# catniplab/vjf

Hardware: AMD Instinct MI355X
Metric: trial-timesteps/sec (higher is better)
Workload: dtype f32

## Files before the change

vjf_amd/csrc/vjf_chol_kernel.h:

```cpp
#pragma once
#include <hip/hip_runtime.h>
#include "vjf_gram_kernel.h"
#include "vjf_plan.h"

#define VJF_CHOL_THREADS 512
#define VJF_CHOL_MAXBLK 7
#define VJF_PREP_ROWS 1

struct VjfPrepArgs {
    float* state;
    const float* red;
    float* gbuf;
    float* aux;
    float* loss4;
    int B_total;
    unsigned flags;
    int n_rowblk, n_sgdblk;
    const unsigned* wait_count;
    unsigned wait_target;
    int bid0;
    const unsigned* run_word; unsigned run_epoch;
    const unsigned* start_count; unsigned start_target;
    unsigned* done_count;
    unsigned* replay_mask; float* replay_rho; int replay_pass;
// ... 569 lines not shown
}

template <int DZP>
__device__ __forceinline__ void vjf_chol_body(const VjfPlan& P, const VjfCholArgs& A, float* lds, int* s_dead, const unsigned it_epoch,
                                              const float* it_red, const unsigned it_wait_target, const unsigned it_stat_target,
                                              const bool it_src_state) {
    int tid = threadIdx.x;
    asm volatile("" : "+v"(tid));
    const int lane = tid & 63, wave = tid >> 6;
    const int n = P.n, dz = P.dz;
    const int nbl = (n + 31) / 32, npad = nbl * 32, ntri = nbl * (nbl + 1) / 2;
    float* S = A.state;
    float* SC = S + P.off[VJF_SLOT_SCALARS];
    const bool do_upd = A.flags & VJF_FLAG_UPDATE, warm = A.flags & VJF_FLAG_WARM_UP;
    if (!do_upd) return;
    if (A.post && warm) return;
    if (A.post && !A.self_prep && tid == 0) __hip_atomic_store(A.flags_out + VJF_CHOL_MAXBLK + 2, it_epoch, __ATOMIC_RELAXED, __HIP_MEMORY_SCOPE_AGENT);
    float* s_blk = lds;
    float* s_aux = s_blk + (size_t)ntri * 1024;
    float* s_g = s_aux + (size_t)nbl * 1024;
    int* s_flag = (int*)(s_g + (size_t)npad * DZP * (DZP <= 16 ? 1 : 2));
    double* s_d = (double*)(s_flag + 8);
    int* s_bi = s_flag + 64;
    int* s_bj = s_bi + 32;

    float* Wm = S + P.off[VJF_SLOT_W_MEAN];
    float* Wc = S + P.off[VJF_SLOT_W_CHOL];
    float* Pm = S + P.off[VJF_SLOT_W_PREC];
    float* Lm = S + P.off[VJF_SLOT_W_PCHOL];
    const float* G = it_red + P.red_G;
    const float* FDX = it_red + P.red_FDX;
    float sig = S[P.off[VJF_SLOT_TR_LOGVAR]];
    const float Bf = (float)A.B_total;
    unsigned st = 0;
    const bool sp = A.post && A.self_prep;
    VJF_STAMP(0);
    if (tid < ntri) {
        int bi = 0;
        while ((bi + 1) * (bi + 2) / 2 <= tid) ++bi;
        s_bi[tid] = bi;
        s_bj[tid] = tid - bi * (bi + 1) / 2;
    }
    if (tid == 0) s_flag[0] = 1;
    if (tid < 16) s_flag[128 + tid] = 0;
    __syncthreads();
    auto stat_wait = [&]() {
        if (A.stat_count && (!vjf_wg_wait_sc1(A.stat_count, it_stat_target, tid, SC + VJF_SC_STATUS, (A.flags & VJF_FLAG_HANDOFF_ACQUIRE) != 0u) || (A.inject_epoch && tid == 0 && it_epoch == A.inject_epoch))) {
            vjf_status_or(SC + VJF_SC_STATUS, VJF_STATUS_RLS_FAILED | VJF_STATUS_WAIT_STATS);
            *s_dead = 1;
        }
    };
    if (warm) stat_wait();

    if (!warm) {
        auto diag_chain = [&](int k) {
            float* dk = s_blk + (size_t)vtri(k, k) * 1024;
            const bool good = potrf_inv_chain2(dk, s_aux + (size_t)k * 1024, lane, min(32, n - 32 * k));
            if (!good && lane == 0) s_flag[0] = 0;
            return good;
        };
        bool chain_good = true;
        auto pad4 = [](int gi, int gj) {
            return make_float4(gi == gj ? 1.f : 0.f, gi == gj + 1 ? 1.f : 0.f, gi == gj + 2 ? 1.f : 0.f, gi == gj + 3 ? 1.f : 0.f);
        };
        bool lscr_guard = false;
        auto sigma_wait = [&]() {
            asm volatile("s_waitcnt vmcnt(0)" ::: "memory");
            __syncthreads();
            if (tid == 0) __hip_atomic_store(A.flags_out + VJF_CHOL_MAXBLK + 2, it_epoch, __ATOMIC_RELAXED, __HIP_MEMORY_SCOPE_AGENT);
            vjf_chaos(tid, A.wait_count, 1);
            if (A.sig_word && it_wait_target != 0u) {
                if (tid == 0) {
                    bool there = false;
                    unsigned bits = 0u;
                    for (unsigned spins = 0; spins < VJF_WAIT_SPINS; ++spins) {
                        const unsigned long long v = __hip_atomic_load(A.sig_word, __ATOMIC_RELAXED, __HIP_MEMORY_SCOPE_AGENT);
                        if ((unsigned)(v >> 32) == it_epoch - 1u) { there = true; bits = (unsigned)v; break; }
                        if ((spins & 255u) == 255u && vjf_abort_seen(SC + VJF_SC_STATUS)) break;
                        __builtin_amdgcn_s_sleep(1);
                    }
                    s_flag[2] = (int)bits; s_flag[3] = there ? 1 : 0;
                }
                __syncthreads();
                sig = __uint_as_float((unsigned)s_flag[2]);
                if (!s_flag[3] && tid == 0) { vjf_status_or(SC + VJF_SC_STATUS, VJF_STATUS_RLS_FAILED | VJF_STATUS_WAIT_SIGMA); *s_dead = 1; }
                lscr_guard = true;
                return;
            }
            if (!vjf_wg_wait_sc1(A.wait_count, it_wait_target, tid, SC + VJF_SC_STATUS, (A.flags & VJF_FLAG_HANDOFF_ACQUIRE) != 0u)) { vjf_status_or(SC + VJF_SC_STATUS, VJF_STATUS_RLS_FAILED | VJF_STATUS_WAIT_SIGMA); *s_dead = 1; }
            sig = __hip_atomic_load(S + P.off[VJF_SLOT_TR_LOGVAR], __ATOMIC_RELAXED, __HIP_MEMORY_SCOPE_AGENT);
        };
        typedef unsigned chol_u4 __attribute__((ext_vector_type(4)));
        const __amdgpu_buffer_rsrc_t r_G = __builtin_amdgcn_make_buffer_rsrc(const_cast<float*>(G), 0, 0x7fffffff, 0x00020000);
        auto g4 = [&](int gi, int gj) {
            if (!(gi < n && gj < n)) return make_float4(0.f, 0.f, 0.f, 0.f);
            if (A.stat_count) {
                const chol_u4 v4 = __builtin_amdgcn_raw_buffer_load_b128(r_G, (gi * n + gj) * 4, 0, 16);
                return make_float4(__uint_as_float(v4[0]), __uint_as_float(v4[1]), __uint_as_float(v4[2]), __uint_as_float(v4[3]));
            }
            return *reinterpret_cast<const float4*>(G + (size_t)gi * n + gj);
        };
        constexpr int NT = VJF_CHOL_THREADS - 64, NQ = ((VJF_CHOL_MAXBLK * (VJF_CHOL_MAXBLK + 1) / 2 - 1) * 256 + NT - 1) / NT;
        const int t2 = tid - 64;
        float4 v[NQ], g[NQ];
        auto idx_of = [&](int q) { return wave == 0 ? (q < 4 ? lane + 64 * q : ntri * 256) : 256 + t2 + q * NT; };
#pragma unroll
        for (int q = 0; q < NQ; ++q) {
            const int idx = idx_of(q);
            v[q] = make_float4(0.f, 0.f, 0.f, 0.f); g[q] = v[q];
            if (idx < ntri * 256) {
                const int b = idx >> 8, r = (idx >> 3) & 31, c4 = (idx & 7) * 4;
                const int gi = s_bi[b] * 32 + r, gj = s_bj[b] * 32 + c4;
                if (sp && !it_src_state) v[q] = *reinterpret_cast<const float4*>(A.pscr + (size_t)idx * 4);
                else v[q] = (gi < n && gj < n) ? *reinterpret_cast<const float4*>(Pm + (size_t)gi * n + gj) : pad4(gi, gj);
            }
        }
        stat_wait();
        if (sp) {
#pragma unroll
            for (int q = 0; q < NQ; ++q) {
                const int idx = idx_of(q);
                if (idx < ntri * 256) {
                    const int b = idx >> 8, r = (idx >> 3) & 31, c4 = (idx & 7) * 4;
                    g[q] = g4(s_bi[b] * 32 + r, s_bj[b] * 32 + c4);
                }
            }
        }
        if (sp) {
            sigma_wait();
            const float inv_v = expf(-sig);
#pragma unroll
            for (int q = 0; q < NQ; ++q) {
                v[q].x = fmaf(g[q].x, inv_v, v[q].x); v[q].y = fmaf(g[q].y, inv_v, v[q].y);
                v[q].z = fmaf(g[q].z, inv_v, v[q].z); v[q].w = fmaf(g[q].w, inv_v, v[q].w);
            }
        }
#pragma unroll
        for (int q = 0; q < NQ; ++q) {
            const int idx = idx_of(q);
            if (idx < ntri * 256) {
                const int b = idx >> 8, r = (idx >> 3) & 31, c4 = (idx & 7) * 4;
                float* blk = s_blk + (size_t)b * 1024;
                blk[vsw(r, c4)] = v[q].x; blk[vsw(r, c4 + 1)] = v[q].y; blk[vsw(r, c4 + 2)] = v[q].z; blk[vsw(r, c4 + 3)] = v[q].w;
                if (A.post) *reinterpret_cast<float4*>(A.pscr + (size_t)idx * 4) = v[q];
            }
        }
        if (wave == 0) chain_good = diag_chain(0);
        else if (!A.post)
            for (int e = t2; e < npad * DZP; e += NT) {
                const int r = e / DZP, j = e - r * DZP;
                s_g[e] = (r < n && j < dz) ? A.gbuf[(size_t)r * dz + j] : 0.f;
            }
        __syncthreads();
        VJF_STAMP(1);

        auto trail = [&](int k, int t) {
            const int bi = k + 1 + s_bi[t], bj = k + 1 + s_bj[t];
            float* cb = s_blk + (size_t)vtri(bi, bj) * 1024;
            vjf_f32x16 acc;
            blk_load(acc, cb, lane);
            blk_mma<true>(acc, s_blk + (size_t)vtri(bi, k) * 1024, s_blk + (size_t)vtri(bj, k) * 1024, -1.f, lane);
            blk_store(acc, cb, lane);
        };
        auto put_block = [&](const float* blk, float* dst, int ld, int gi0, int gj0, bool lower_only) {
#pragma unroll
            for (int q = 0; q < 4; ++q) {
                const int idx = lane + 64 * q, r = idx >> 3, c4 = (idx & 7) * 4;
                vjf_f32x4 o;
                o[0] = (!lower_only || c4 <= r) ? blk[vsw(r, c4)] : 0.f;
                o[1] = (!lower_only || c4 + 1 <= r) ? blk[vsw(r, c4 + 1)] : 0.f;
                o[2] = (!lower_only || c4 + 2 <= r) ? blk[vsw(r, c4 + 2)] : 0.f;
                o[3] = (!lower_only || c4 + 3 <= r) ? blk[vsw(r, c4 + 3)] : 0.f;
                if (gi0 + r < ld && gj0 + c4 < ld) {
                    float* p = dst + (size_t)(gi0 + r) * ld + gj0 + c4;
                    asm volatile("global_store_dwordx4 %0, %1, off sc1\n\ts_nop 1" ::"v"(p), "v"(o) : "memory");
                }
            }
        };
        auto publish = [&](int k0, int k1, unsigned fail) {
            vjf_chaos(lane, A.flags_out + k0, 2);
            asm volatile("s_waitcnt vmcnt(0)" ::: "memory");
            if (lane >= k0 && lane < k1) __hip_atomic_store(A.flags_out + lane, (it_epoch << 1) | fail, __ATOMIC_RELAXED, __HIP_MEMORY_SCOPE_AGENT);
        };
        volatile int* s_ctl = s_flag + 128;
        enum { C_CHAIN = 0, C_P1 = 1, C_A = 2, C_B = 3, C_HB = 4 };
        volatile int* v_ok = s_flag;
        auto lds_wait = [&](int w, int target) {
            for (unsigned spins = 0; spins < (1u << 22); ++spins) {
                if (s_ctl[w] >= target || !v_ok[0]) break;
                __builtin_amdgcn_s_sleep(1);
            }
            if (s_ctl[w] < target && v_ok[0]) v_ok[0] = 0;
            __builtin_amdgcn_fence(__ATOMIC_ACQUIRE, "workgroup");
        };
        auto lds_post = [&](int w, int v) {
            __builtin_amdgcn_fence(__ATOMIC_RELEASE, "workgroup");
            if (lane == 0) s_ctl[w] = v;
        };
        auto hb_arrive = [&](int hw, int stages_done) {
            __builtin_amdgcn_fence(__ATOMIC_RELEASE, "workgroup");
            if (lane == 0) s_ctl[C_HB + hw] = stages_done;
        };
        auto hb_wait = [&](int stages_done) {
            for (unsigned spins = 0; spins < (1u << 22); ++spins) {
                int lo = s_ctl[C_HB];
#pragma unroll
                for (int h2 = 1; h2 < 6; ++h2) lo = min(lo, (int)s_ctl[C_HB + h2]);
                if (lo >= stages_done || !v_ok[0]) break;
                __builtin_amdgcn_s_sleep(1);
            }
            __builtin_amdgcn_fence(__ATOMIC_ACQUIRE, "workgroup");
        };
        auto panel_tile = [&](int bi, int k) {
            float* pb = s_blk + (size_t)vtri(bi, k) * 1024;
            vjf_f32x16 acc;
#pragma unroll
            for (int r = 0; r < 16; ++r) acc[r] = 0.f;
            blk_mma<true>(acc, pb, s_aux + (size_t)k * 1024, 1.f, lane);
            blk_store(acc, pb, lane);
        };
        auto trail_tile = [&](int bi, int bj, int k) {
            float* cb = s_blk + (size_t)vtri(bi, bj) * 1024;
            vjf_f32x16 acc;
            blk_load(acc, cb, lane);
            blk_mma<true>(acc, s_blk + (size_t)vtri(bi, k) * 1024, s_blk + (size_t)vtri(bj, k) * 1024, -1.f, lane);
            blk_store(acc, cb, lane);
        };
        int kdone = 0;
        if (wave == 0) {
            auto wait_ab = [&](int target) {
// ... 341 lines not shown
```

vjf_amd/csrc/vjf_mega_kernel.h:

```cpp
#pragma once
#include <hip/hip_runtime.h>
#include "vjf_chol_kernel.h"
#include "vjf_plan.h"
#include "vjf_post_kernel.h"
#include "vjf_trial_mfma_kernel.h"
#include "vjf_act.h"

#define VJF_MG_THREADS 512
#define VJF_MG_WAVES 8
#define VJF_MG_TR 32
#define VJF_MG_LD 33
#define VJF_MG_GROWS 96
#define VJF_MG_MAXQ 4
#define VJF_MG_RING 32
#define VJF_MG_TAG_TILES 512
#define RS_RESID 5

#ifndef MG_C_SPREAD
#define MG_C_SPREAD 1
#endif
enum {
    MG_C_FWD = 16 * MG_C_SPREAD,
    MG_C_K1 = 32 * MG_C_SPREAD,
    MG_C_BWD = 48 * MG_C_SPREAD,
// ... 759 lines not shown
                v2a += __shfl_xor(v2a, 16, 64); v2a += __shfl_xor(v2a, 32, 64);
                v2b += __shfl_xor(v2b, 16, 64); v2b += __shfl_xor(v2b, 32, 64);
                if (lane < 16) { s_red[wave * TR + lane] = v2a; s_red[wave * TR + 16 + lane] = v2b; }
                if (wave < nsl) {
                    const int sl = msl;
                    vjf_f32x4 acc0 = {0.f, 0.f, 0.f, 0.f}, acc1 = {0.f, 0.f, 0.f, 0.f};
                    if (mpre) { if (mke > mkb) mg_mma2_mm16(acc0, acc1, am, s_phi, dz, 0, mkb, mke, 0, lane); }
                    else mg_mma2(acc0, acc1, Wm, dz, dz, 0, s_phi, mkb, mke, lane);
                    float* pr = s_part + (size_t)(sl * 16 + 4 * (lane >> 4)) * LD + (lane & 15);
#pragma unroll
                    for (int r = 0; r < 4; ++r) { pr[r * LD] = acc0[r]; pr[r * LD + 16] = acc1[r]; }
                }
                mean_nsl = nsl;
            }
            __syncthreads(); MG_PHASE();
            };
            auto moments_b = [&]() {
            if (!replay) {
                if (tid < TR) {
                    float v = 0.f;
                    for (int w = 0; w < NW; ++w) v += s_red[w * TR + tid];
                    s_plv[tid] = logf(v);
                }
                for (int e = tid; e < TR * dz; e += NT) {
                    const int j = e >> 5, b = e & 31;
                    float v = 0.f;
                    for (int sl = 0; sl < mean_nsl; ++sl) v += s_part[(size_t)(sl * 16 + j) * LD + b];
                    s_pm[j * LD + b] = s_xu[j * LD + b] + v;
                    if (want_resid) s_dmu[j * LD + b] = v;
                }
            }
            __syncthreads(); MG_PHASE();
            };
            if (!RLS && !replay && first && !use_mom) { mg_warm(A.xt, P.n * P.n, wg, tid); mg_warm(S + P.off[VJF_SLOT_W_MEAN], (P.n * P.dz) & ~3, wg, tid); }
            if (!RLS && !replay && !use_mom) { moments_a(); moments_b(); }
            if (!RLS && !replay && first) VJF_MG_STAMPW(2);
            if (first && !replay) {
                if (gated) gate();
                if (gated && t > 0 && vjf_abort_wg()) return;
                if (want_replay) break;
                if (t > 0 && !tl) {
                    mg_warm(A.aux, P.aux_len, wg, tid);
                    mg_warm(S + P.train_off, P.train_len, wg, tid);
                }
            }
            float4 wv[2];
            const bool warm_now = first && !replay && rls_now && !rls_in;
            if (first && !replay) rho = mg_ld(S + P.off[VJF_SLOT_LIK_LOGVAR]);
            if (first && !replay && !mode_rls) sig = mg_ld(S + P.off[VJF_SLOT_TR_LOGVAR]);
            if (warm_now) {
                mg_warm_issue(A.xt, P.n * P.n, wg, tid, wv);
                sig = mg_ld(S + P.off[VJF_SLOT_TR_LOGVAR]);
                tri = mg_ld(SCW + VJF_SC_TRI_CLEAN) != 0.f;
                rls_in = true;
            }
            if (first && tl && !replay && t == 0) {
                if (!vjf_wg_wait_sc1<RLS ? VJF_POLL_SLEEP : VJF_POLL_SLEEP_LITE>(cnt + MG_C_IMG, (unsigned)A.n_sgd, tid, SCW + VJF_SC_STATUS, (A.flags & VJF_FLAG_HANDOFF_ACQUIRE) != 0u))
                    vjf_status_or(SCW + VJF_SC_STATUS, VJF_STATUS_RLS_FAILED | VJF_STATUS_WAIT_GATE);
                if (vjf_abort_wg()) return;
            }
            if (first && tl && !replay && (gated || t == 0)) {
                const __amdgpu_buffer_rsrc_t r_img = mg_rsrc(A.img);
                float4* dst = reinterpret_cast<float4*>(smem + Lo.th0);
                const int n4 = Lo.th_len >> 2;
                for (int q0 = tid; q0 < n4; q0 += 8 * NT) {
                    float4 v[8];
#pragma unroll
                    for (int q = 0; q < 8; ++q) if (q0 + q * NT < n4) v[q] = mg_ld4(r_img, (q0 + q * NT) * 4);
#pragma unroll
                    for (int q = 0; q < 8; ++q) if (q0 + q * NT < n4) dst[q0 + q * NT] = v[q];
                }
                __syncthreads(); MG_PHASE();
            }
            if (warm_now) mg_warm_retire(wv);
            if (first) { VJF_MG_STAMP(1); VJF_MG_STAMPX(27, -1); VJF_MG_STAMPW(0); }
            if (first && A.stamps && tid == 0 && t == A.T - 1 && !replay) {
                unsigned xcc;
                unsigned hwid;
                asm volatile("s_getreg_b32 %0, hwreg(HW_REG_XCC_ID)" : "=s"(xcc));
                asm volatile("s_getreg_b32 %0, hwreg(HW_REG_HW_ID)" : "=s"(hwid));
                A.stamps[1024 + (size_t)wg * 8 + 6] = (xcc & 15u) | ((unsigned long long)hwid << 8);
                A.stamps[1024 + (size_t)wg * 8 + 7] = rls_in ? 1u : 0u;
            }
            {
                const float* xin = s_in;
                int kin = din, aoff = 0;
                for (int l = 0; l < P.L; ++l) {
                    const float* WT = A.aux + P.aux_recT[l];
                    int th_w = 0, th_ldw = 0, th_b = 0;
                    if (tl) mg_theta_layer(P, Lo.th0, l, th_w, th_ldw, th_b);
                    const float* bias_l = smem + th_b; const float* bias_g = S + P.off[VJF_SLOT_REC_B0 + 2 * l];
                    float* out = s_act + aoff * LD;
                    const int hl = P.h[l], mt = (hl + 15) >> 4;
                    for (int tt = wave; tt < mt; tt += NW) {
                        vjf_f32x4 acc0 = {0.f, 0.f, 0.f, 0.f}, acc1 = {0.f, 0.f, 0.f, 0.f};
                        if (tl) mg_mma2_lds<false>(acc0, acc1, smem + th_w, th_ldw, hl, tt * 16, xin, 0, kin, lane);
                        else mg_mma2(acc0, acc1, WT, hl, hl, tt * 16, xin, 0, kin, lane);
#pragma unroll
                        for (int r = 0; r < 4; ++r) {
                            const int f = tt * 16 + 4 * (lane >> 4) + r;
                            if (f < hl) {
                                const float bf = tl ? ((mg_lds_cf*)bias_l)[f] : ((mg_glb_cf*)bias_g)[f];
                                if (ACT) {
                                    out[f * LD + (lane & 15)] = vjf_act_fwd(act, acc0[r] + bf);
                                    out[f * LD + 16 + (lane & 15)] = vjf_act_fwd(act, acc1[r] + bf);
                                } else {
                                    out[f * LD + (lane & 15)] = mg_tanh(acc0[r] + bf);
                                    out[f * LD + 16 + (lane & 15)] = mg_tanh(acc1[r] + bf);
                                }
                            }
                        }
                    }
                    __syncthreads(); MG_PHASE();
                    xin = out; kin = hl; aoff += hl;
                }
                if (first) VJF_MG_STAMP(23);
                const float* HT = A.aux + P.aux_headT;
                const int mt = (2 * dz + 15) >> 4;
                const int nsl = min(NW / mt, part_rows / (16 * mt));
                if (wave < mt * nsl) {
                    const int tt = wave / nsl, sl = wave - tt * nsl;
                    const int per = (((kin + 3) >> 2) + nsl - 1) / nsl * 4;
                    vjf_f32x4 acc0 = {0.f, 0.f, 0.f, 0.f}, acc1 = {0.f, 0.f, 0.f, 0.f};
                    if (tl) mg_mma2_lds<false>(acc0, acc1, smem + Lo.th_head, Lo.th_ldh, 2 * dz, tt * 16, xin, sl * per, min(kin, (sl + 1) * per), lane);
                    else mg_mma2(acc0, acc1, HT, 2 * dz, 2 * dz, tt * 16, xin, sl * per, min(kin, (sl + 1) * per), lane);
                    float* pr = s_part + (size_t)((sl * mt + tt) * 16 + 4 * (lane >> 4)) * LD + (lane & 15);
#pragma unroll
                    for (int r = 0; r < 4; ++r) { pr[r * LD] = acc0[r]; pr[r * LD + 16] = acc1[r]; }
                }
                __syncthreads(); MG_PHASE();
                if (first) VJF_MG_STAMP(24);
                const float* bl_l = smem + Lo.th_bl; const float* bl_g = S + P.off[VJF_SLOT_LV_B];
                for (int e = tid; e < TR * 2 * dz; e += NT) {
                    const int f = e >> 5, b = e & 31;
                    float v = 0.f;
                    for (int sl = 0; sl < nsl; ++sl) v += s_part[(size_t)((sl * mt + (f >> 4)) * 16 + (f & 15)) * LD + b];
                    if (f < dz) s_mu[f * LD + b] = v; else s_lv[(f - dz) * LD + b] = v + (tl ? ((mg_lds_cf*)bl_l)[f - dz] : ((mg_glb_cf*)bl_g)[f - dz]);
                }
            }
            __syncthreads(); MG_PHASE();
            if (first) VJF_MG_STAMP(3);
            for (int e = tid; e < TR * dz; e += NT) {
                const int j = e >> 5, b = e & 31;
                const float xt = fmaf(s_e2[j * LD + b], expf(0.5f * s_lv[j * LD + b]), s_mu[j * LD + b]);
                s_xt[j * LD + b] = xt;
                s_dx[j * LD + b] = b < nb ? xt - s_xu[j * LD + b] : 0.f;
            }
            if (!replay) {
                float* mrow = mu_t + (size_t)b0 * dz;
                float* lrow = lv_t + (size_t)b0 * dz;
                const int ne = nb * dz;
                const int n4 = ((((size_t)mrow | (size_t)lrow) & 15u) == 0) ? (ne >> 2) : 0;
                for (int e4 = tid; e4 < n4; e4 += NT) {
                    float vm[4], vl[4];
#pragma unroll
                    for (int c = 0; c < 4; ++c) {
                        const int e = 4 * e4 + c, b = mg_div(e, m_dz), j = e - b * dz;
                        vm[c] = s_mu[j * LD + b]; vl[c] = s_lv[j * LD + b];
                    }
                    mg_st4(mrow + 4 * e4, vm[0], vm[1], vm[2], vm[3]);
                    mg_st4(lrow + 4 * e4, vl[0], vl[1], vl[2], vl[3]);
                }
                for (int e = 4 * n4 + tid; e < ne; e += NT) {
                    const int b = mg_div(e, m_dz), j = e - b * dz;
                    mg_st(mrow + e, s_mu[j * LD + b]);
                    mg_st(lrow + e, s_lv[j * LD + b]);
                }
            }
            __syncthreads(); MG_PHASE();
            {
                constexpr int LPT = NT / TR;
                const int b = tid / LPT, sl = tid % LPT;
                float sdx2 = 0.f;
                for (int j = sl; j < dz; j += LPT) { const float dx = s_dx[j * LD + b]; sdx2 = fmaf(dx, dx, sdx2); }
                sdx2 = group_sum<LPT>(sdx2);
                if (sl == 0) s_sc[b * RS_N + RS_SDX2] = sdx2;
            }
            {
                const float* CT = A.aux + P.aux_decT;
                const float* d_l = smem + Lo.th_bd; const float* d_g = S + P.off[VJF_SLOT_DEC_B];
                const int mt = (dy + 15) >> 4;
                for (int tt = wave; tt < mt; tt += NW) {
                    vjf_f32x4 acc0 = {0.f, 0.f, 0.f, 0.f}, acc1 = {0.f, 0.f, 0.f, 0.f};
                    if (tl) mg_mma2_lds<false>(acc0, acc1, smem + Lo.th_dec, Lo.th_ldd, dy, tt * 16, s_xt, 0, dz, lane);
                    else mg_mma2(acc0, acc1, CT, dy, dy, tt * 16, s_xt, 0, dz, lane);
#pragma unroll
                    for (int r = 0; r < 4; ++r) {
                        const int f = tt * 16 + 4 * (lane >> 4) + r;
                        if (f < dy) { const float df = tl ? ((mg_lds_cf*)d_l)[f] : ((mg_glb_cf*)d_g)[f]; s_py[f * LD + (lane & 15)] = acc0[r] + df; s_py[f * LD + 16 + (lane & 15)] = acc1[r] + df; }
                    }
                }
            }
            if (first) VJF_MG_STAMP(25);
            if (!replay && mode_rls) {
                const int mt = (n + 15) >> 4;
                for (int tt = NW - 1 - wave; tt < mt; tt += NW) {
                    const int m0 = tt * 16, i = lane & 15, kk = lane >> 4;
                    const float* arow = ((m0 + i) < n ? s_phi + (size_t)(m0 + i) * LD : s_zero) + kk;
                    const float* brow = (i < dz ? s_dx + (size_t)i * LD : s_zero) + kk;
                    float a[8], b[8];
#pragma unroll
                    for (int s = 0; s < 8; ++s) { a[s] = arow[4 * s]; b[s] = brow[4 * s]; }
                    vjf_f32x4 acc = {0.f, 0.f, 0.f, 0.f}, acc1 = {0.f, 0.f, 0.f, 0.f};
#pragma unroll
                    for (int s = 0; s < 8; s += 2) {
                        acc = __builtin_amdgcn_mfma_f32_16x16x4f32(a[s], b[s], acc, 0, 0, 0);
                        acc1 = __builtin_amdgcn_mfma_f32_16x16x4f32(a[s + 1], b[s + 1], acc1, 0, 0, 0);
                    }
                    acc += acc1;
                    const int fq = m0 + 4 * (lane >> 4), col = lane & 15;
                    if (col < dz && fq < ldn) {
                        float* p = early + (size_t)col * ldn + fq;
                        if (!first) { acc[0] += mg_ld(p); acc[1] += mg_ld(p + 1); acc[2] += mg_ld(p + 2); acc[3] += mg_ld(p + 3); }
                        mg_st4(p, acc[0], acc[1], acc[2], acc[3]);
                    }
                }
            }
            if (tid == 0 && first && last && !replay && !rls_in)
                s_wg[15] = ((int)(__hip_atomic_load(cnt + MG_C_PDONE, __ATOMIC_RELAXED, __HIP_MEMORY_SCOPE_AGENT) - (unsigned)t * npost) >= 0) ? 1.f : 0.f;
            if (use_mom && !replay) asm volatile("s_waitcnt vmcnt(0)" ::: "memory");
            __syncthreads(); MG_PHASE();
            if (use_mom && !replay && tid == 0) __hip_atomic_store(cnt + MG_C_TAG_POST + tile, (unsigned)(tc + 1), __ATOMIC_RELAXED, __HIP_MEMORY_SCOPE_AGENT);
            float touch = 0.f;
            if (!gated && !replay && last && tc + 1 < A.T) {
                const int tn = wg;
                const int b0n = tn * TR, nbn = min(TR, A.B - b0n);
                const int ly = (nbn * dy + 31) / 32 + 1, le = (nbn * dz + 31) / 32 + 1;
                const float* yn = A.y + (size_t)(tc + 1) * sy + (size_t)b0n * dy;
                const float* en = A.eps + (size_t)(tc + 1) * 2 * sz + (size_t)b0n * dz;
                const float* tp = nullptr;
                if (tid < ly) tp = yn + min(tid * 32, nbn * dy - 1);
                else if (tid < ly + le) tp = en + min((tid - ly) * 32, nbn * dz - 1);
                else if (tid < ly + 2 * le) tp = en + sz + min((tid - ly - le) * 32, nbn * dz - 1);
                if (tp) touch = *tp;
            }
            if (tid == 0 && !replay && mode_rls) {
                float v = 0.f;
                for (int bb = 0; bb < TR; ++bb) v += s_sc[bb * RS_N + RS_SDX2];
                s_wg[RS_SDX2] += v;
                if (last) mg_st(early + (size_t)16 * ldn + RS_SDX2, s_wg[RS_SDX2]);
            }
            if (first) VJF_MG_STAMP(26);
            const bool fuse_fwd = first && last && !replay && !rls_in && s_wg[15] != 0.f;
            if (last && !replay && !fuse_fwd && mode_rls) vjf_wg_signal_wt(cnt + MG_C_FWD, tid);
            if (first) VJF_MG_STAMP(4);
            if (last) { VJF_MG_STAMPX(28, -1); VJF_MG_STAMPW(1); }
            float4 wv_late[2];
            bool warm_late = false;
            if (first && !rls_in) {
                if (!vjf_wg_wait_sc1<RLS ? VJF_POLL_SLEEP : VJF_POLL_SLEEP_LITE>(cnt + MG_C_PDONE, (unsigned)t * npost, tid, SCW + VJF_SC_STATUS, (A.flags & VJF_FLAG_HANDOFF_ACQUIRE) != 0u))
                    vjf_status_or(SCW + VJF_SC_STATUS, VJF_STATUS_RLS_FAILED | VJF_STATUS_WAIT_K1);
                if (vjf_abort_wg()) return;
                sig = mg_ld(S + P.off[VJF_SLOT_TR_LOGVAR]);
                tri = mg_ld(SCW + VJF_SC_TRI_CLEAN) != 0.f;
                if (fuse_fwd) {
                    vjf_chaos(tid, cnt + MG_C_FWD, 2);
                    asm volatile("s_waitcnt vmcnt(0)" ::: "memory");
                    __syncthreads();
                    if (tid == 0) __hip_atomic_fetch_add(cnt + MG_C_FWD, 1u, __ATOMIC_RELAXED, __HIP_MEMORY_SCOPE_AGENT);
                }
                mg_warm_issue(A.xt, P.n * P.n, wg, tid, wv_late);
                warm_late = true;
            }
            if (first) { VJF_MG_STAMP(5); if (RLS) VJF_MG_STAMPW(2); }
            if (use_mom && !replay) {
                if (!vjf_wg_wait_sc1<RLS ? VJF_POLL_SLEEP : VJF_POLL_SLEEP_LITE>(cnt + MG_C_TAG_MOM + tile, (unsigned)(tc + 1), tid, SCW + VJF_SC_STATUS, (A.flags & VJF_FLAG_HANDOFF_ACQUIRE) != 0u))
                    vjf_status_or(SCW + VJF_SC_STATUS, VJF_STATUS_RLS_FAILED | VJF_STATUS_WAIT_K1);
                if (vjf_abort_wg()) return;
                const float* mb = A.mom + ((size_t)tile * 2 + (size_t)(tc & 1)) * (size_t)((2 * dz + 1) * TR);
                for (int e = tid; e < TR * (2 * dz + 1); e += NT) {
                    const int j = e >> 5, b = e & 31;
                    const float v = mg_ld(mb + e);
                    if (j < dz) s_pm[j * LD + b] = v;
                    else if (j < 2 * dz) { if (want_resid) s_dmu[(j - dz) * LD + b] = v; }
                    else s_plv[b] = v;
                }
                __syncthreads(); MG_PHASE();
            }
            asm volatile("" ::"v"(touch));
            if (RLS) moments_a();
            if (warm_late) mg_warm_retire(wv_late);
            if (last && tid == 0 && !replay && mode_rls) __hip_atomic_fetch_add(cnt + MG_C_K1, 1u, __ATOMIC_RELAXED, __HIP_MEMORY_SCOPE_AGENT);
            if (RLS) moments_b();
            if (do_sgd)
            for (int e = tid; e < TR * (dz + 1); e += NT) {
                const int j = e >> 5, b = e & 31;
                if (b < nb) {
                    float* sv = A.pmsave + (size_t)(b0 + b) * (dz + 1) + j;
                    if (!replay) *sv = j < dz ? s_pm[j * LD + b] : s_plv[b];
                    else if (j < dz) s_pm[j * LD + b] = *sv;
                    else s_plv[b] = *sv;
                }
            }
            if (replay) { __syncthreads(); MG_PHASE(); }
            if (first) VJF_MG_STAMP(10);
            if (first) { VJF_MG_STAMP(6); VJF_MG_STAMPW(3); }
            {
                constexpr int LPT = NT / TR;
                const int b = tid / LPT, s = tid % LPT;
                const bool ok = b < nb;
                float lrec = 0.f, ssey = 0.f;
                if (P.lik == VJF_LIK_GAUSSIAN) {
                    const float p = expf(-0.5f * rho), e = expf(-rho);
                    for (int i = s; i < dy; i += LPT) {
                        const float yv = s_in[i * LD + b], pv = s_py[i * LD + b];
                        const float r = pv - yv, dsc = yv * p - pv * p;
                        lrec += 0.5f * (dsc * dsc + rho);
                        ssey = fmaf(r, r, ssey);
                        s_dpy[i * LD + b] = (ok && m_r) ? e * r : 0.f;
                    }
                } else {
                    for (int i = s; i < dy; i += LPT) {
                        const float yv = s_in[i * LD + b], pv = s_py[i * LD + b];
                        const float eta = fminf(pv, 10.f), ex = expf(eta);
                        lrec += ex - yv * eta;
                        const float r = pv - yv;
                        ssey = fmaf(r, r, ssey);
                        s_dpy[i * LD + b] = (ok && m_r && pv <= 10.f) ? (ex - yv) : 0.f;
                    }
                }
                lrec = group_sum<LPT>(lrec);
                ssey = group_sum<LPT>(ssey);
                float ldyn = 0.f, ent = 0.f, rsd = 0.f;
                {
                    const float p = expf(-0.5f * sig), e = expf(-sig), plv = s_plv[b];
                    for (int j = s; j < dz; j += LPT) {
                        const float mp = s_pm[j * LD + b], mu = s_mu[j * LD + b], lv = s_lv[j * LD + b];
                        if (want_resid) { const float r = s_dx[j * LD + b] - s_dmu[j * LD + b]; rsd = fmaf(r, r, rsd); }
                        const float dsc = mp * p - mu * p;
                        const float tr = expf(plv + lv - sig);
                        ldyn += 0.5f * (dsc * dsc + sig) + 0.5f * tr;
                        ent += 0.5f * lv;
                        float dmu = 0.f, dlv = m_h ? -0.5f : 0.f;
                        if (!warm && m_d) { dmu = -e * (mp - mu); dlv += 0.5f * tr; }
                        s_dmu[j * LD + b] = ok ? dmu : 0.f;
                        s_dlv[j * LD + b] = ok ? dlv : 0.f;
                    }
                }
                ldyn = group_sum<LPT>(ldyn);
                ent = group_sum<LPT>(ent);
                if (want_resid) rsd = group_sum<LPT>(rsd);
                if (s == 0) {
                    s_sc[b * RS_N + RS_RESID] = ok ? rsd : 0.f;
                    s_sc[b * RS_N + RS_LRECON] = ok ? lrec : 0.f;
                    s_sc[b * RS_N + RS_LDYN] = ok ? ldyn : 0.f;
                    s_sc[b * RS_N + RS_ENT] = ok ? ent : 0.f;
// ... 1119 lines not shown
```

vjf_amd/csrc/vjf_post_kernel.h:

```cpp
#pragma once
#include <hip/hip_runtime.h>
#include "vjf_plan.h"
#include "vjf_chol_kernel.h"
#include "vjf_trial_mfma_kernel.h"

#define VJF_SPIN_LIMIT VJF_WAIT_SPINS
#define VJF_POST_THREADS 512
#define VJF_POST_KPAR 4
#define VJF_POST_LDB 33
#define VJF_POST_LDX 17
#define VJF_RESID_BLOCKS 64

struct VjfPostArgs {
    float* state;
    const float* dinv;
    const float* lscr;
    const float* gbuf;
    const unsigned* flags;
    unsigned epoch;
    float* status;
    const unsigned* k1_done;
    unsigned k1_target;
    unsigned* started;
    unsigned* done;
// ... 394 lines not shown
    auto store_W = [&]() {
        float* Wm = A.state + P.off[VJF_SLOT_W_MEAN];
        for (int e = tid; e < n * 16; e += VJF_POST_THREADS) {
            const int r = e >> 4, c = e & 15;
            if (c < dz) __hip_atomic_store(Wm + r * dz + c, s_x[r * LX + c], __ATOMIC_RELAXED, __HIP_MEMORY_SCOPE_AGENT);
        }
    };
    if (!failed && !k1_late) store_W();
    if (!A.fold_sigma) { leave(); return; }
    {
        double* s_p = reinterpret_cast<double*>(lds);
        if (failed) {
            wait_g();
            if (tid == 0) { __builtin_amdgcn_fence(__ATOMIC_ACQUIRE, "agent"); asm volatile("s_waitcnt vmcnt(0)" ::: "memory"); }
            __syncthreads();
            const float* Wold = A.state + P.off[VJF_SLOT_W_MEAN];
            for (int e = tid; e < nbl * 32 * 16; e += VJF_POST_THREADS) {
                const int r = e >> 4, c = e & 15;
                s_x[r * LX + c] = (r < n && c < dz) ? Wold[(size_t)r * dz + c] : 0.f;
            }
            prefetch_tail();
            if (A.undo_P) {
                float* Pm = A.state + P.off[VJF_SLOT_W_PREC];
                const float* G = it_red + P.red_G;
                const float inv_v = expf(-S[P.off[VJF_SLOT_TR_LOGVAR]]);
                for (int e = tid; e < n * n; e += VJF_POST_THREADS) vjf_store_wt(Pm + e, fmaf(-G[e], inv_v, Pm[e]));
            }
        }
        __syncthreads();
        VJF_POST_STAMP(20);
#ifdef VJF_EXPERIMENT_SLOW_RLS
        { const unsigned long long t0_ = wall_clock64(); while (wall_clock64() - t0_ < VJF_EXPERIMENT_SLOW_RLS) __builtin_amdgcn_s_sleep(1); }
#endif
        double part = 0.0;
        const int c = lane & 31, h = lane >> 5;
#pragma unroll
        for (int q = 0; q < 4; ++q) {
            const int t = wave + 8 * q;
            if (t < ntri) {
                const int code = s_tab[32 + t], bi = code >> 8, bj = code & 255;
                vjf_f32x16 acc;
#pragma unroll
                for (int r = 0; r < 16; ++r) acc[r] = 0.f;
                float wa[8], wb[8];
#pragma unroll
                for (int k = 0; k < 8; ++k) {
                    wa[k] = s_x[(bi * 32 + c) * LX + 2 * k + h];
                    wb[k] = s_x[(bj * 32 + c) * LX + 2 * k + h];
                }
#pragma unroll
                for (int k = 0; k < 8; ++k)
                    if (2 * k < dz) acc = __builtin_amdgcn_mfma_f32_32x32x2f32(wa[k], wb[k], acc, 0, 0, 0);
                double tp = 0.0;
#pragma unroll
                for (int r = 0; r < 16; ++r) {
                    const float wgt = (float)((wbits[q] >> (2 * r)) & 3u);
                    tp += (double)((wgt * gpre[q][r]) * acc[r]);
                }
                part += tp;
            }
        }
#pragma unroll
        for (int q = 0; q < 8; ++q) {
            const int e = tid + q * VJF_POST_THREADS, r = e >> 4, cc = e & 15;
            if (r < n && cc < dz) part -= 2.0 * (double)s_x[r * LX + cc] * (double)fpre[q];
        }

#pragma unroll
        for (int o = 32; o > 0; o >>= 1) part += __shfl_xor(part, o, 64);
        if (lane == 0) s_p[wave] = part;
        __syncthreads();
        if (tid == 0) {
            double t = 0.0;
            for (int w = 0; w < VJF_POST_THREADS / 64; ++w) t += s_p[w];
            t += (double)pre_sdx2;
            if (t < 0.0) t = 0.0;
            float* St = A.state;
            float* SC = St + P.off[VJF_SLOT_SCALARS];
            const float mse = (float)(t * pre_scale);
            const float new_sig = logf(pre_old + ((float)A.B_total / pre_tot) * mse);
            if (A.sig_word)
                __hip_atomic_store(A.sig_word, ((unsigned long long)it_epoch << 32) | (unsigned long long)__float_as_uint(new_sig), __ATOMIC_RELAXED,
                                   __HIP_MEMORY_SCOPE_AGENT);
            bool ok1 = true;
            if (k1_late && A.k1_done) {
                ok1 = false;
                for (unsigned spins = 0; spins < VJF_SPIN_LIMIT; ++spins) {
                    const unsigned v = __hip_atomic_load(A.k1_done, __ATOMIC_RELAXED, __HIP_MEMORY_SCOPE_AGENT);
                    if ((int)(v - it_k1_target) >= 0) { ok1 = true; break; }
                    if ((spins & 255u) == 255u && vjf_abort_seen(A.status)) break;
                    __builtin_amdgcn_s_sleep(4);
                }
                if (!ok1) { vjf_status_or(A.status, VJF_STATUS_RLS_FAILED | VJF_STATUS_WAIT_COLUMN); *s_dead = 1; }
            }
            s_ctl[0] = ok1 ? 1 : 0;
            if (ok1) {
                __hip_atomic_store(St + P.off[VJF_SLOT_TR_LOGVAR], new_sig, __ATOMIC_RELAXED, __HIP_MEMORY_SCOPE_AGENT);
                __hip_atomic_store(SC + VJF_SC_N_TR, pre_tot, __ATOMIC_RELAXED, __HIP_MEMORY_SCOPE_AGENT);
            }
            if (failed) vjf_status_or(SC + VJF_SC_STATUS, VJF_STATUS_RLS_FAILED);
        }
        VJF_POST_STAMP(21);
        if (k1_late) {
            __syncthreads();
            if (s_ctl[0] && !failed) store_W();
        }
    }
    leave();
}

__device__ __forceinline__ void vjf_rls_post_loop(const VjfPlan& P, const VjfPostArgs& A, float* lds, int* s_dead, const int role, const int bix) {
    const int steps = A.nsteps > 0 ? A.nsteps : 1;
    if (A.xt && role == 1) {
        const int n = P.n, nwg = 2 * ((n + 31) / 32);
        const float* Wc = A.state + P.off[VJF_SLOT_W_CHOL];
        for (int e = bix * VJF_POST_THREADS + (int)threadIdx.x; e < n * n; e += nwg * VJF_POST_THREADS) {
            const int k = e / n, j = e - k * n;
            vjf_store_wt(A.xt + (size_t)j * n + k, Wc[e]);
        }
        vjf_wg_signal_wt(A.xt_count, (int)threadIdx.x);
    }
    for (int it = 0; it < steps; ++it) {
        const float* red = ((A.step0 + it) & 1) ? A.red2 : A.red;
        vjf_rls_post_body(P, A, lds, s_dead, A.epoch + (unsigned)it, red, A.k1_target + (unsigned)it * A.k1_stride,
                          A.prep_target + (unsigned)it * A.prep_stride, it == 0, role, bix);
        __syncthreads();
        if (*s_dead) break;
    }
}

__global__ __launch_bounds__(VJF_POST_THREADS) void vjf_rls_post_kernel(VjfPlan P, VjfPostArgs A) {
    extern __shared__ __attribute__((aligned(16))) float lds[];
    __shared__ int s_dead;
    if (threadIdx.x == 0) s_dead = 0;
    __syncthreads();
    vjf_rls_post_loop(P, A, lds, &s_dead, A.role, (int)blockIdx.x);
}

template <int DZP>
__global__ __launch_bounds__(VJF_CHOL_THREADS) void vjf_rls_pair_kernel(VjfPlan P, VjfCholArgs C, VjfPostArgs Q) {
    static_assert(VJF_CHOL_THREADS == VJF_POST_THREADS, "one workgroup size for both halves");
    extern __shared__ __attribute__((aligned(16))) float lds[];
    __shared__ int s_dead;
    if (threadIdx.x == 0) s_dead = 0;
    __syncthreads();
    if (blockIdx.x == 0) vjf_chol_loop<DZP>(P, C, lds, &s_dead);
    else if (blockIdx.x == 1) vjf_rls_post_loop(P, Q, lds, &s_dead, 2, 0);
    else vjf_rls_post_loop(P, Q, lds, &s_dead, 1, (int)blockIdx.x - 2);
}



__global__ __launch_bounds__(64) void vjf_gate_kernel(const unsigned* count, unsigned target, float* status) {
    if (threadIdx.x != 0) return;
    for (unsigned spins = 0; spins < VJF_SPIN_LIMIT; ++spins) {
        const unsigned v = __hip_atomic_load(count, __ATOMIC_RELAXED, __HIP_MEMORY_SCOPE_AGENT);
        if ((int)(v - target) >= 0) return;
        if ((spins & 255u) == 255u && vjf_abort_seen(status)) return;
        __builtin_amdgcn_s_sleep(2);
    }
    vjf_status_or(status, VJF_STATUS_RLS_FAILED | VJF_STATUS_WAIT_GATE);
}

__global__ __launch_bounds__(64) void vjf_count_kernel(unsigned* count) {
    if (threadIdx.x == 0) __hip_atomic_fetch_add(count, 1u, __ATOMIC_RELEASE, __HIP_MEMORY_SCOPE_AGENT);
}
// ... 109 lines not shown
```

Measured before the change: 78.52 million.

## Poll post-done counter early in mega kernel to skip forward-handoff wait

Adds a lookahead check of the post-kernel done counter at two points in the first tile's forward pass. If the previous step's post work is already complete, the workgroup loads sigma and the tri flag directly, marks rls_in, and skips waiting on the RLS handoff. The old fused forward-signal path is removed, so the FWD signal is now always issued. It also adds timing stamps in the chol and post kernels. The aim is to cut synchronisation stalls between the RLS/post stage and the next timestep, at the cost of extra atomic polls and a changed handoff protocol.

```diff
diff --git a/vjf_amd/csrc/vjf_chol_kernel.h b/vjf_amd/csrc/vjf_chol_kernel.h
--- a/vjf_amd/csrc/vjf_chol_kernel.h
+++ b/vjf_amd/csrc/vjf_chol_kernel.h
@@ -675,6 +675,7 @@
                     s_flag[2] = (int)bits; s_flag[3] = there ? 1 : 0;
                 }
                 __syncthreads();
+                VJF_STAMP(23);
                 sig = __uint_as_float((unsigned)s_flag[2]);
                 if (!s_flag[3] && tid == 0) { vjf_status_or(SC + VJF_SC_STATUS, VJF_STATUS_RLS_FAILED | VJF_STATUS_WAIT_SIGMA); *s_dead = 1; }
                 lscr_guard = true;
@@ -738,7 +739,7 @@
                 if (A.post) *reinterpret_cast<float4*>(A.pscr + (size_t)idx * 4) = v[q];
             }
         }
-        if (wave == 0) chain_good = diag_chain(0);
+        if (wave == 0) { VJF_STAMP(24); chain_good = diag_chain(0); VJF_STAMP(25); }
         else if (!A.post)
             for (int e = t2; e < npad * DZP; e += NT) {
                 const int r = e / DZP, j = e - r * DZP;
diff --git a/vjf_amd/csrc/vjf_mega_kernel.h b/vjf_amd/csrc/vjf_mega_kernel.h
--- a/vjf_amd/csrc/vjf_mega_kernel.h
+++ b/vjf_amd/csrc/vjf_mega_kernel.h
@@ -865,6 +865,14 @@
                 A.stamps[1024 + (size_t)wg * 8 + 6] = (xcc & 15u) | ((unsigned long long)hwid << 8);
                 A.stamps[1024 + (size_t)wg * 8 + 7] = rls_in ? 1u : 0u;
             }
+            const bool look = RLS && first && !replay && !rls_in && t > 0;
+            bool seen = false;
+            auto look_issue = [&]() -> unsigned {
+                vjf_chaos(tid, cnt + MG_C_PDONE, 1);
+                return __hip_atomic_load(cnt + MG_C_PDONE, __ATOMIC_RELAXED, __HIP_MEMORY_SCOPE_AGENT);
+            };
+            auto pdone_there = [&](unsigned v) { return (int)(v - (unsigned)t * npost) >= 0; };
+            unsigned look_v = 0u;
             {
                 const float* xin = s_in;
                 int kin = din, aoff = 0;
@@ -898,6 +906,7 @@
                     xin = out; kin = hl; aoff += hl;
                 }
                 if (first) VJF_MG_STAMP(23);
+                if (look && tid == 0) look_v = look_issue();
                 const float* HT = A.aux + P.aux_headT;
                 const int mt = (2 * dz + 15) >> 4;
                 const int nsl = min(NW / mt, part_rows / (16 * mt));
@@ -911,7 +920,9 @@
 #pragma unroll
                     for (int r = 0; r < 4; ++r) { pr[r * LD] = acc0[r]; pr[r * LD + 16] = acc1[r]; }
                 }
+                if (look && tid == 0) s_wg[14] = pdone_there(look_v) ? 1.f : 0.f;
                 __syncthreads(); MG_PHASE();
+                if (look && s_wg[14] != 0.f) seen = true;
                 if (first) VJF_MG_STAMP(24);
                 const float* bl_l = smem + Lo.th_bl; const float* bl_g = S + P.off[VJF_SLOT_LV_B];
                 for (int e = tid; e < TR * 2 * dz; e += NT) {
@@ -975,6 +986,7 @@
                 }
             }
             if (first) VJF_MG_STAMP(25);
+            if (look && !seen && tid == 0) look_v = look_issue();
             if (!replay && mode_rls) {
                 const int mt = (n + 15) >> 4;
                 for (int tt = NW - 1 - wave; tt < mt; tt += NW) {
@@ -999,10 +1011,17 @@
                     }
                 }
             }
-            if (tid == 0 && first && last && !replay && !rls_in)
-                s_wg[15] = ((int)(__hip_atomic_load(cnt + MG_C_PDONE, __ATOMIC_RELAXED, __HIP_MEMORY_SCOPE_AGENT) - (unsigned)t * npost) >= 0) ? 1.f : 0.f;
+            if (look && !seen && tid == 0) s_wg[15] = pdone_there(look_v) ? 1.f : 0.f;
             if (use_mom && !replay) asm volatile("s_waitcnt vmcnt(0)" ::: "memory");
             __syncthreads(); MG_PHASE();
+            if (look && !seen && s_wg[15] != 0.f) seen = true;
+            if (look && A.stamps && tid == 0 && t == A.T - 1)
+                A.stamps[1024 + (size_t)wg * 8 + 7] = seen ? (s_wg[14] != 0.f ? 2u : 3u) : 0u;
+            if (seen) {
+                sig = mg_ld(S + P.off[VJF_SLOT_TR_LOGVAR]);
+                tri = mg_ld(SCW + VJF_SC_TRI_CLEAN) != 0.f;
+                rls_in = true;
+            }
             if (use_mom && !replay && tid == 0) __hip_atomic_store(cnt + MG_C_TAG_POST + tile, (unsigned)(tc + 1), __ATOMIC_RELAXED, __HIP_MEMORY_SCOPE_AGENT);
             float touch = 0.f;
             if (!gated && !replay && last && tc + 1 < A.T) {
@@ -1024,8 +1043,7 @@
                 if (last) mg_st(early + (size_t)16 * ldn + RS_SDX2, s_wg[RS_SDX2]);
             }
             if (first) VJF_MG_STAMP(26);
-            const bool fuse_fwd = first && last && !replay && !rls_in && s_wg[15] != 0.f;
-            if (last && !replay && !fuse_fwd && mode_rls) vjf_wg_signal_wt(cnt + MG_C_FWD, tid);
+            if (last && !replay && mode_rls) vjf_wg_signal_wt(cnt + MG_C_FWD, tid);
             if (first) VJF_MG_STAMP(4);
             if (last) { VJF_MG_STAMPX(28, -1); VJF_MG_STAMPW(1); }
             float4 wv_late[2];
@@ -1036,15 +1054,9 @@
                 if (vjf_abort_wg()) return;
                 sig = mg_ld(S + P.off[VJF_SLOT_TR_LOGVAR]);
                 tri = mg_ld(SCW + VJF_SC_TRI_CLEAN) != 0.f;
-                if (fuse_fwd) {
-                    vjf_chaos(tid, cnt + MG_C_FWD, 2);
-                    asm volatile("s_waitcnt vmcnt(0)" ::: "memory");
-                    __syncthreads();
-                    if (tid == 0) __hip_atomic_fetch_add(cnt + MG_C_FWD, 1u, __ATOMIC_RELAXED, __HIP_MEMORY_SCOPE_AGENT);
-                }
-                mg_warm_issue(A.xt, P.n * P.n, wg, tid, wv_late);
                 warm_late = true;
             }
+            if (warm_late || seen) { mg_warm_issue(A.xt, P.n * P.n, wg, tid, wv_late); warm_late = true; }
             if (first) { VJF_MG_STAMP(5); if (RLS) VJF_MG_STAMPW(2); }
             if (use_mom && !replay) {
                 if (!vjf_wg_wait_sc1<RLS ? VJF_POLL_SLEEP : VJF_POLL_SLEEP_LITE>(cnt + MG_C_TAG_MOM + tile, (unsigned)(tc + 1), tid, SCW + VJF_SC_STATUS, (A.flags & VJF_FLAG_HANDOFF_ACQUIRE) != 0u))
diff --git a/vjf_amd/csrc/vjf_post_kernel.h b/vjf_amd/csrc/vjf_post_kernel.h
--- a/vjf_amd/csrc/vjf_post_kernel.h
+++ b/vjf_amd/csrc/vjf_post_kernel.h
@@ -500,6 +500,7 @@
             if (A.sig_word)
                 __hip_atomic_store(A.sig_word, ((unsigned long long)it_epoch << 32) | (unsigned long long)__float_as_uint(new_sig), __ATOMIC_RELAXED,
                                    __HIP_MEMORY_SCOPE_AGENT);
+            VJF_POST_STAMP(26);
             bool ok1 = true;
             if (k1_late && A.k1_done) {
                 ok1 = false;
```

Result: slower. 77.67 million, median of 2 (-1.1%).
